# sauloal/pykmer

Measured on AMD Instinct MI355X. Metric: bp/s k-mer counted (k=15, 1 GPU), higher is better.
Workload: dtype u8; 1 GPU; k=15 canonical k-mer count of one 800 Mbp synthetic genome per GPU (SURVEY 8d C2, seed 2+rank), 4^15 table resident in HBM; fasta_bytes=813333854, num_kmers=766212116, parallelism=1 independent genome(s)

## Files before the change

### include/pykmer_hip.h

```cpp
#ifndef PYKMER_HIP_H
#define PYKMER_HIP_H

#include <stddef.h>
#include <stdint.h>

#ifdef __cplusplus
extern "C" {
#endif

#define PK_ABI_VERSION 3

enum {
    PK_OK = 0,
    PK_ERR_ARG = -1,
    PK_ERR_HIP = -2,
    PK_ERR_RECS_CAP = -3,
    PK_ERR_STATE = -4,
    PK_ERR_FORMAT = -5
};

#define PK_FORMAT_FASTA 0
#define PK_FORMAT_FASTQ 1

typedef struct pk_record {
// ... 114 lines not shown
int pk_trim_set_cover(pk_trim *t, const uint8_t *cover, uint64_t n_bases, int min_qual_byte);
int pk_trim_feed(pk_trim *t, const uint8_t *host_text, uint64_t n_bytes, const uint64_t *starts, uint64_t n_records, uint64_t *out);
int pk_trim_feed_device(pk_trim *t, const void *dev_text, uint64_t n_bytes, const uint64_t *starts, uint64_t n_records, uint64_t *out);
int pk_trim_finish(pk_trim *t, uint64_t totals_out[3]);
int pk_trim_timings(pk_trim *t, double out[2]);
void pk_trim_destroy(pk_trim *t);

enum { PK_CORR_POS2 = 0, PK_CORR_SEQ_LEN = 1, PK_CORR_CANDIDATES = 2, PK_CORR_UNTRIED = 3, PK_CORR_CORRECTED = 4, PK_CORR_AMBIGUOUS = 5,
       PK_CORR_FIELDS = 6 };
typedef struct pk_correct pk_correct;
int pk_correct_create(pk_correct **out, int k, int device);
int pk_correct_set_tables(pk_correct *c, const void *const *dev_tables, int N, int min_count, int max_count);
int pk_correct_set_cover(pk_correct *c, const uint8_t *cover, uint64_t n_bases, int min_qual_byte, int min_windows);
int pk_correct_feed(pk_correct *c, const uint8_t *host_text, uint64_t n_bytes, const uint64_t *starts, uint64_t n_records,
                    uint8_t *host_text_out, uint64_t *out);
int pk_correct_feed_device(pk_correct *c, const void *dev_text, uint64_t n_bytes, const uint64_t *starts, uint64_t n_records,
                           void *dev_text_out, uint64_t *out);
int pk_correct_finish(pk_correct *c, uint64_t totals_out[6]);
int pk_correct_timings(pk_correct *c, double out[2]);
void pk_correct_destroy(pk_correct *c);

int pk_bgzf_scan(const uint8_t *src, uint64_t n_bytes, uint64_t cap, uint64_t *c_off_out, uint64_t *c_size_out,
                 uint64_t *isize_out, uint64_t *n_blocks_out);
int pk_bgzf_inflate(const uint8_t *src, uint64_t src_bytes, const uint64_t *c_off, const uint64_t *c_size,
                    const uint64_t *u_off, uint64_t n_blocks, uint8_t *dst, int threads);
int pk_bgzf_deflate(const uint8_t *src, uint64_t n_bytes, int level, uint32_t block_input, uint8_t *dst, uint64_t dst_cap,
                    uint64_t *c_sizes_out, uint64_t *total_out, int threads);

int pk_diag_occupancy(int which);
int pk_diag_plan(int k, uint64_t n_bytes, uint64_t out[8]);
int pk_diag_settled_chunks(pk_indexer *ix, uint64_t *out);
int pk_diag_plan_slice(int k, int n_slices, uint64_t n_bytes, uint64_t out[16]);
int pk_diag_level2_order(const uint32_t *sizes, uint32_t B1, uint32_t *order_out);

#ifdef __cplusplus
}
#endif
#endif
```

### pykmer_amd/_lib.py

```python
import ctypes
import os

import numpy as np

_HERE = os.path.dirname(os.path.abspath(__file__))
from ._rt import LIB_PATH, open_library

PK_OK, PK_ERR_ARG, PK_ERR_HIP, PK_ERR_RECS_CAP, PK_ERR_STATE, PK_ERR_FORMAT = 0, -1, -2, -3, -4, -5
PK_FORMAT_FASTA, PK_FORMAT_FASTQ = 0, 1
FORMATS = {"fasta": PK_FORMAT_FASTA, "fastq": PK_FORMAT_FASTQ}
MASK_HARD, MASK_INVERT = 1, 2

RECORD_DTYPE = np.dtype([("name_off", "<u8"), ("name_len", "<u8"), ("seq_len", "<u8"), ("n_valid_kmers", "<u8")])

_u64p = ctypes.POINTER(ctypes.c_uint64)
_SIGNATURES = {
    "pk_version": (ctypes.c_int, []),
    "pk_last_error": (ctypes.c_int, [ctypes.c_char_p, ctypes.c_size_t]),
    "pk_device_count": (ctypes.c_int, []),
    "pk_warm": (ctypes.c_int, [ctypes.c_int]),
    "pk_dev_alloc": (ctypes.c_int, [ctypes.POINTER(ctypes.c_void_p), ctypes.c_uint64, ctypes.c_int]),
    "pk_dev_free": (ctypes.c_int, [ctypes.c_void_p, ctypes.c_int]),
    "pk_dev_upload": (ctypes.c_int, [ctypes.c_void_p, ctypes.c_void_p, ctypes.c_uint64, ctypes.c_int]),
    "pk_dev_download": (ctypes.c_int, [ctypes.c_void_p, ctypes.c_void_p, ctypes.c_uint64, ctypes.c_int]),
# ... 66 lines not shown
    "pk_select_set_records": (ctypes.c_int, [ctypes.c_void_p, ctypes.c_void_p, ctypes.c_void_p, ctypes.c_uint64]),
    "pk_select_feed": (ctypes.c_int, [ctypes.c_void_p, ctypes.c_void_p, ctypes.c_uint64, ctypes.c_void_p, ctypes.c_uint64, _u64p]),
    "pk_select_feed_device": (ctypes.c_int, [ctypes.c_void_p, ctypes.c_void_p, ctypes.c_uint64, ctypes.c_void_p, ctypes.c_uint64, _u64p]),
    "pk_select_finish": (ctypes.c_int, [ctypes.c_void_p, ctypes.c_void_p]),
    "pk_select_timings": (ctypes.c_int, [ctypes.c_void_p, ctypes.c_void_p]),
    "pk_select_destroy": (None, [ctypes.c_void_p]),
    "pk_trim_create": (ctypes.c_int, [ctypes.POINTER(ctypes.c_void_p), ctypes.c_int]),
    "pk_trim_set_cover": (ctypes.c_int, [ctypes.c_void_p, ctypes.c_void_p, ctypes.c_uint64, ctypes.c_int]),
    "pk_trim_feed": (ctypes.c_int, [ctypes.c_void_p, ctypes.c_void_p, ctypes.c_uint64, ctypes.c_void_p, ctypes.c_uint64, ctypes.c_void_p]),
    "pk_trim_feed_device": (ctypes.c_int, [ctypes.c_void_p, ctypes.c_void_p, ctypes.c_uint64, ctypes.c_void_p, ctypes.c_uint64, ctypes.c_void_p]),
    "pk_trim_finish": (ctypes.c_int, [ctypes.c_void_p, ctypes.c_void_p]),
    "pk_trim_timings": (ctypes.c_int, [ctypes.c_void_p, ctypes.c_void_p]),
    "pk_trim_destroy": (None, [ctypes.c_void_p]),
    "pk_correct_create": (ctypes.c_int, [ctypes.POINTER(ctypes.c_void_p), ctypes.c_int, ctypes.c_int]),
    "pk_correct_set_tables": (ctypes.c_int, [ctypes.c_void_p, ctypes.c_void_p, ctypes.c_int, ctypes.c_int, ctypes.c_int]),
    "pk_correct_set_cover": (ctypes.c_int, [ctypes.c_void_p, ctypes.c_void_p, ctypes.c_uint64, ctypes.c_int, ctypes.c_int]),
    "pk_correct_feed": (ctypes.c_int, [ctypes.c_void_p, ctypes.c_void_p, ctypes.c_uint64, ctypes.c_void_p, ctypes.c_uint64, ctypes.c_void_p,
                                        ctypes.c_void_p]),
    "pk_correct_feed_device": (ctypes.c_int, [ctypes.c_void_p, ctypes.c_void_p, ctypes.c_uint64, ctypes.c_void_p, ctypes.c_uint64, ctypes.c_void_p,
                                               ctypes.c_void_p]),
    "pk_correct_finish": (ctypes.c_int, [ctypes.c_void_p, ctypes.c_void_p]),
    "pk_correct_timings": (ctypes.c_int, [ctypes.c_void_p, ctypes.c_void_p]),
    "pk_correct_destroy": (None, [ctypes.c_void_p]),
    "pk_bgzf_scan": (ctypes.c_int, [ctypes.c_void_p, ctypes.c_uint64, ctypes.c_uint64, ctypes.c_void_p, ctypes.c_void_p, ctypes.c_void_p, _u64p]),
    "pk_bgzf_inflate": (ctypes.c_int, [ctypes.c_void_p, ctypes.c_uint64, ctypes.c_void_p, ctypes.c_void_p, ctypes.c_void_p, ctypes.c_uint64, ctypes.c_void_p,
                                        ctypes.c_int]),
    "pk_bgzf_deflate": (ctypes.c_int, [ctypes.c_void_p, ctypes.c_uint64, ctypes.c_int, ctypes.c_uint32, ctypes.c_void_p, ctypes.c_uint64,
                                        ctypes.c_void_p, _u64p, ctypes.c_int]),
    "pk_diag_occupancy": (ctypes.c_int, [ctypes.c_int]),
    "pk_diag_plan": (ctypes.c_int, [ctypes.c_int, ctypes.c_uint64, ctypes.c_void_p]),
    "pk_diag_settled_chunks": (ctypes.c_int, [ctypes.c_void_p, _u64p]),
    "pk_diag_plan_slice": (ctypes.c_int, [ctypes.c_int, ctypes.c_int, ctypes.c_uint64, ctypes.c_void_p]),
    "pk_diag_level2_order": (ctypes.c_int, [ctypes.c_void_p, ctypes.c_uint32, ctypes.c_void_p]),
}
EXPORTS = tuple(_SIGNATURES)

_lib = None


class PkError(RuntimeError):
    def __init__(self, code, message):
        super().__init__(f"libpykmer_hip error {code}: {message}")
        self.code = code


def load():
    global _lib
    if _lib is None:
        lib = open_library()
        for name, (res, args) in _SIGNATURES.items():
            fn = getattr(lib, name)
            fn.restype, fn.argtypes = res, args
        _lib = lib
    return _lib


def _check(rc):
    if rc != PK_OK:
        buf = ctypes.create_string_buffer(512)
        load().pk_last_error(buf, 512)
        msg = buf.value.decode("utf-8", "replace")
        if rc == PK_ERR_ARG:
            raise ValueError(msg)
        raise PkError(rc, msg)


# ... 646 lines not shown
                                  ctypes.byref(total), int(threads)))
    return dst[: total.value], sizes[:n_blocks].astype(np.int64)


def diag_plan(k: int, n_bytes: int = 0) -> dict:
    out = np.zeros(8, dtype=np.uint64)
    _check(load().pk_diag_plan(k, n_bytes, out.ctypes.data))
    names = ("feed_max", "capacity1", "capacity2", "B1", "B2", "fb_bits", "n_chunks", "fits_u32")
    return {n: int(v) for n, v in zip(names, out)}


WS_VARIANTS = ("narrow", "narrow_sliced", "k15", "k17", "wide_sliced", "deep", "wide")
COUNT_KERNELS = ("whole", "bytes", "half")


def diag_plan_slice(k: int, n_slices: int = 1, n_bytes: int = 0) -> dict:
    out = np.zeros(16, dtype=np.uint64)
    _check(load().pk_diag_plan_slice(k, n_slices, n_bytes, out.ctypes.data))
    names = ("addr_bits", "fb_bits", "b1", "b2", "sample_stride", "n_tally", "sample2", "n_chunks", "variant", "count_kernel",
             "split", "B1", "B2", "capacity1", "capacity2", "fits_u32")
    d = {n: int(v) for n, v in zip(names, out)}
    d["variant"] = WS_VARIANTS[d["variant"]]
    d["count_kernel"] = COUNT_KERNELS[d["count_kernel"]]
    return d


def diag_level2_order(sizes) -> np.ndarray:
    s = np.ascontiguousarray(sizes, dtype=np.uint32)
    out = np.zeros(max(1, s.size), dtype=np.uint32)
    _check(load().pk_diag_level2_order(s.ctypes.data, s.size, out.ctypes.data))
    return out[:s.size]


def gram_expand(pair: np.ndarray) -> np.ndarray:
    p = np.ascontiguousarray(pair, dtype=np.uint64)
    N = p.shape[0]
    m = np.zeros((N, N, 3), dtype=np.uint64)
    _check(load().pk_gram_expand(p.ctypes.data, N, m.ctypes.data))
    return m
```

### pykmer_amd/csrc/kmer_part.hip

```cpp
#include <cstddef>
#include <string>
#include <type_traits>
#include "../../include/pykmer_hip.h"
#include "part_common.h"

namespace pk {

int set_error(int code, const std::string &msg);

__global__ __launch_bounds__(1024) void k_sample2(const uint32_t *__restrict__ in, const uint32_t *__restrict__ bucket_base,
                                                  const uint32_t *__restrict__ bucket_end, PartPlan pl, uint32_t stride2,
                                                  uint32_t *__restrict__ tally, uint32_t *__restrict__ sampled_n,
                                                  const uint32_t *__restrict__ flags) {
    __shared__ uint32_t h[512];
    __shared__ uint32_t n_seen;
    if (flags[0]) return;
    const uint32_t b = blockIdx.x, lo = bucket_base[b], hi = bucket_end[b];
    if (threadIdx.x < 512) h[threadIdx.x] = 0;
    if (threadIdx.x == 0) n_seen = 0;
    __syncthreads();
    const uint32_t n_grp = (hi - lo + 255u) / 256u, n_sgrp = (n_grp + stride2 - 1u) / stride2;
    const uint32_t mask = pl.B2 - 1u, shift = pl.fb_bits, w = threadIdx.x >> 6, lane = threadIdx.x & 63u;
    uint32_t mine = 0;
    for (uint32_t s0 = 0; s0 < n_sgrp; s0 += 8u * 16u) {
// ... 138 lines not shown
            }
            const bool full = v_lo == win && n_tile == (uint32_t)TILE;
            uint32_t okm = 0;
            if (!full) {
#pragma unroll
                for (int j = 0; j < PER / 4; j++) {
                    const uint32_t i = win + (threadIdx.x + j * NT) * 4u;
#pragma unroll
                    for (int e = 0; e < 4; e++) okm |= (i + e >= v_lo && i + e < v_hi) ? (1u << (j * 4 + e)) : 0u;
                }
            }
            if (win + TILE < hi) fetch(win + TILE, nxt);
            uint32_t *cl = cursor + (uint64_t)b * B;
            const uint32_t *ce = cap_end + (uint64_t)b * B;
            if (full) scatter_tile<uint32_t, false, NT, PER, 512, true, 8, REC24>(L, r, 0u, n_tile, shift, B, low_mask, true, out, settle, cl, ce, dump, flags);
            else scatter_tile<uint32_t, false, NT, PER, 512, false, 8, REC24>(L, r, okm, n_tile, shift, B, low_mask, true, out, settle, cl, ce, dump, flags);
        }
    };
    const uint32_t *pos = wg2_start;
    const uint32_t per = pl.B1 >> 3;
    const uint32_t o_lo = (blockIdx.x & 7u) * per, o_hi = o_lo + per, first = blockIdx.x >> 3, step = gridDim.x >> 3;
    const uint32_t w_end = pos[o_hi];
    for (uint32_t w = pos[o_lo] + first; w < w_end; w += step) {
        uint32_t a = o_lo, z = o_hi;
        while (z - a > 1) { const uint32_t m = (a + z) >> 1; if (pos[m] <= w) a = m; else z = m; }
        const uint32_t b = l2_order[a];
        const uint64_t s = (uint64_t)bucket_base[b] + (uint64_t)(w - pos[a]) * pl.R2;
        const uint64_t e = min(s + pl.R2, (uint64_t)bucket_end[b]);
        item(b, (uint32_t)s, (uint32_t)e);
    }
}

constexpr uint32_t K6_PIECE = 65024;
constexpr int K6_BYTES_LDS = 65536 + 1024 + 128;

__device__ __forceinline__ int wave_sum_i32(int v) {
    v += __builtin_amdgcn_update_dpp(0, v, 0x128, 0xf, 0xf, false);
    v += __builtin_amdgcn_update_dpp(0, v, 0x124, 0xf, 0xf, false);
    v += __builtin_amdgcn_update_dpp(0, v, 0x122, 0xf, 0xf, false);
    v += __builtin_amdgcn_update_dpp(0, v, 0x121, 0xf, 0xf, false);
    return __builtin_amdgcn_readlane(v, 0) + __builtin_amdgcn_readlane(v, 16) + __builtin_amdgcn_readlane(v, 32) +
           __builtin_amdgcn_readlane(v, 48);
}

typedef unsigned short U16x2 __attribute__((ext_vector_type(2)));
__device__ __forceinline__ uint32_t clamp255_pair(uint32_t x) {
    const U16x2 lim = {255, 255};
    return __builtin_bit_cast(uint32_t, __builtin_elementwise_min(__builtin_bit_cast(U16x2, x), lim));
}
__device__ __forceinline__ uint32_t pack_low_bytes(uint32_t x0, uint32_t x1) {
    return __builtin_amdgcn_perm(x1, x0, 0x06040200u);
}

struct SliceTally {
    int d1 = 0, d2 = 0;
    __device__ __forceinline__ void add_dword(int *dh, uint32_t x, int sign) {
        uint32_t p0 = x & 0x01010101u, p1 = (x >> 1) & 0x01010101u;
        uint32_t rest = p0 & p1;
        const uint32_t high = x & 0xfcfcfcfcu;
        if (high) {
            const uint32_t big = (((high & 0x7f7f7f7fu) + 0x7f7f7f7fu) | high) & 0x80808080u;
            const uint32_t keep = ~(big >> 7);
            p0 &= keep; p1 &= keep;
            rest = (p0 & p1) | (big >> 7);
        }
        const int n1 = (int)__builtin_popcount(p0 & ~p1), n2 = (int)__builtin_popcount(p1 & ~p0);
        d1 += sign * n1; d2 += sign * n2;
        while (rest) {
            const int bit = __ffs(rest) - 1;
            atomicAdd(&dh[(x >> bit) & 0xffu], sign);
            rest &= rest - 1u;
        }
    }
};

template <int T, bool LEAN, bool NOREC = false>
__device__ __forceinline__ void bucket_count_body(const uint16_t *__restrict__ recs, const uint32_t *__restrict__ final_start,
                                                  const uint32_t *__restrict__ final_end, uint32_t fb_bits, uint32_t split_bits,
                                                  uint8_t *__restrict__ table8, uint32_t fresh, unsigned long long *__restrict__ hist_rep, uint8_t *smem,
                                                  int *dh, uint32_t wg) {
    uint32_t *cnt = reinterpret_cast<uint32_t *>(smem);
    const uint32_t fb = wg >> split_bits, part = wg & ((1u << split_bits) - 1u);
    const uint32_t start = final_start[fb], end = final_end ? final_end[fb] : final_start[fb + 1];
    const uint32_t part_bits = fb_bits - split_bits;
    const uint32_t n_addr = 1u << part_bits;
    uint8_t *slice = table8 + ((uint64_t)fb << fb_bits) + (uint64_t)part * n_addr;
    if (start == end) {
        if (fresh) {
            if (n_addr >= 16) for (uint32_t g = threadIdx.x; g < n_addr / 16; g += T) reinterpret_cast<uint4 *>(slice)[g] = make_uint4(0, 0, 0, 0);
            else for (uint32_t a = threadIdx.x; a < n_addr; a += T) slice[a] = 0;
        }
        return;
    }
    const uint32_t base = start & ~7u;
    const uint32_t i_first = base + threadIdx.x * 8;
    uint4 v_first = make_uint4(0, 0, 0, 0);
    if (i_first < min(base + K6_PIECE, end)) v_first = *reinterpret_cast<const uint4 *>(recs + i_first);
    const bool by_rec = NOREC ? false : (((end - start) >> split_bits) < n_addr / 4 || n_addr < 16);
    SliceTally tally;
    for (uint32_t i = threadIdx.x; i < 256; i += T) dh[i] = 0;
    if (fresh) {
        if (n_addr >= 8) for (uint32_t g = threadIdx.x; g < n_addr / 8; g += T) reinterpret_cast<uint4 *>(cnt)[g] = make_uint4(0, 0, 0, 0);
        else for (uint32_t a = threadIdx.x; a < max(n_addr / 2, 1u); a += T) cnt[a] = 0u;
    } else if (n_addr >= 16) {
        if (!by_rec) __syncthreads();
        for (uint32_t g = threadIdx.x; g < n_addr / 16; g += T) {
            uint4 v = reinterpret_cast<const uint4 *>(slice)[g];
            uint32_t w[4] = {v.x, v.y, v.z, v.w};
            if (!by_rec) {
#pragma unroll
                for (int q = 0; q < 4; q++) tally.add_dword(dh, w[q], -1);
            }
#pragma unroll
            for (int q = 0; q < 8; q++)
                cnt[g * 8 + q] = __builtin_amdgcn_perm(0u, w[q >> 1], (q & 1) ? 0x0c030c02u : 0x0c010c00u);
        }
    } else {
        for (uint32_t a = threadIdx.x; a < max(n_addr / 2, 1u); a += T) cnt[a] = slice[2 * a] | (n_addr > 1u ? (uint32_t)slice[2 * a + 1] << 16 : 0u);
    }
    __syncthreads();
    auto bump = [&](uint32_t a, uint32_t n) {
        const uint32_t sh = 16u * (a & 1u);
        if (!by_rec) { atomicAdd(&cnt[a >> 1], n << sh); return; }
        int &d1 = tally.d1, &d2 = tally.d2;
        const uint32_t c = (atomicAdd(&cnt[a >> 1], n << sh) >> sh) & 0xffffu;
        const uint32_t oc = c > 255u ? 255u : c, nc = c + n > 255u ? 255u : c + n;
        if (oc == nc) return;
        if (nc == 1u) d1++;
        else if (nc == 2u && oc == 1u) { d2++; d1--; }
        else {
            atomicAdd(&dh[nc], 1);
            if (oc) atomicAdd(&dh[oc], -1);
        }
    };
    auto count8 = [&](const uint4 &v, uint32_t i) {
        const uint32_t w[4] = {v.x, v.y, v.z, v.w};
        if (LEAN && !by_rec) {
            const bool interior = i >= start && i + 8u <= end;
            uint8_t *cb = reinterpret_cast<uint8_t *>(cnt);
#pragma unroll
            for (int q = 0; q < 8; q++) {
                const uint32_t x = w[q >> 1];
                const uint32_t off = (q & 1) ? ((x >> 15) & 0x1fffcu) : ((x << 1) & 0x1fffcu);
                const uint32_t low = (q & 1) ? ((x >> 16) & 1u) : (x & 1u);
                uint32_t val = low * 0xffffu + 1u;
                if (!interior) val = (i + q >= start && i + q < end) ? val : 0u;
                __hip_atomic_fetch_add(reinterpret_cast<uint32_t *>(cb + off), val, __ATOMIC_RELAXED, __HIP_MEMORY_SCOPE_WORKGROUP);
            }
            return;
// ... 34 lines not shown
            else if (c == 1u) { tally.d2++; tally.d1--; }
            else { atomicAdd(&dh[c + 1u], 1); atomicAdd(&dh[c], -1); }
        }
    };
    constexpr int NIT = (K6_PIECE + T * 8 - 1) / (T * 8);
    if (end - base <= (uint32_t)T * 8u) {
        if (i_first < end) { if (by_rec) count8_sparse(v_first, i_first); else count8(v_first, i_first); }
        __syncthreads();
    } else {
        for (uint32_t p0 = base; p0 < end; p0 += K6_PIECE) {
            const uint32_t p1 = min(p0 + K6_PIECE, end);
            uint4 v[NIT];
#pragma unroll
            for (int it = 0; it < NIT; it++) {
                const uint32_t i = p0 + (threadIdx.x + it * T) * 8;
                v[it] = make_uint4(0, 0, 0, 0);
                if (i < p1) v[it] = (it == 0 && p0 == base) ? v_first : *reinterpret_cast<const uint4 *>(recs + i);
            }
#pragma unroll
            for (int it = 0; it < NIT; it++) {
                const uint32_t i = p0 + (threadIdx.x + it * T) * 8;
                if (i < p1) count8(v[it], i);
            }
            __syncthreads();
            if (p1 < end) {
                for (uint32_t a = threadIdx.x; a < max(n_addr / 2, 1u); a += T) {
                    cnt[a] = clamp255_pair(cnt[a]);
                }
                __syncthreads();
            }
        }
    }
    if (n_addr >= 16) {
        for (uint32_t g = threadIdx.x; g < n_addr / 16; g += T) {
            const uint4 c0 = reinterpret_cast<const uint4 *>(cnt)[g * 2], c1 = reinterpret_cast<const uint4 *>(cnt)[g * 2 + 1];
            const uint32_t o[4] = {pack_low_bytes(clamp255_pair(c0.x), clamp255_pair(c0.y)), pack_low_bytes(clamp255_pair(c0.z), clamp255_pair(c0.w)),
                                   pack_low_bytes(clamp255_pair(c1.x), clamp255_pair(c1.y)), pack_low_bytes(clamp255_pair(c1.z), clamp255_pair(c1.w))};
            if (!by_rec) {
#pragma unroll
                for (int q = 0; q < 4; q++) tally.add_dword(dh, o[q], 1);
            }
            reinterpret_cast<uint4 *>(slice)[g] = make_uint4(o[0], o[1], o[2], o[3]);
        }
    } else {
        for (uint32_t a = threadIdx.x; a < max(n_addr / 2, 1u); a += T) {
            uint32_t x = cnt[a], lo = x & 0xffffu, hi = x >> 16;
            slice[2 * a] = (uint8_t)(lo > 255u ? 255u : lo);
            if (n_addr > 1u) slice[2 * a + 1] = (uint8_t)(hi > 255u ? 255u : hi);
        }
    }
    const int d1 = wave_sum_i32(tally.d1), d2 = wave_sum_i32(tally.d2);
    if ((threadIdx.x & 63) == 0) {
        if (d1) atomicAdd(&dh[1], d1);
        if (d2) atomicAdd(&dh[2], d2);
    }
    __syncthreads();
    for (uint32_t i = threadIdx.x; i < 256; i += T) {
        const int v = dh[i];
        if (v) atomicAdd(&hist_rep[(uint64_t)(blockIdx.x % HIST_REPLICAS) * 256 + i], (unsigned long long)(long long)v);
    }
}

template <int T>
__global__ __launch_bounds__(T) void k_bucket_count(const uint16_t *__restrict__ recs, const uint32_t *__restrict__ final_start,
                                                    const uint32_t *__restrict__ final_end, uint32_t fb_bits, uint32_t split_bits,
                                                    uint8_t *__restrict__ table8, uint32_t fresh, unsigned long long *__restrict__ hist_rep,
                                                    const uint32_t *__restrict__ flags) {
    extern __shared__ __attribute__((aligned(16))) uint8_t smem[];
    __shared__ int dh[256];
    if (flags[0]) return;
    bucket_count_body<T, true>(recs, final_start, final_end, fb_bits, split_bits, table8, fresh, hist_rep, smem, dh, blockIdx.x);
}
template <int T, bool FRESH>
__global__ __launch_bounds__(T) __attribute__((amdgpu_waves_per_eu(8, 8)))
void k_bucket_count_half_lean(const uint16_t *__restrict__ recs, const uint32_t *__restrict__ final_start, const uint32_t *__restrict__ final_end,
                              uint32_t fb_bits, uint32_t split_bits, uint8_t *__restrict__ table8, uint32_t fresh, unsigned long long *__restrict__ hist_rep,
                              const uint32_t *__restrict__ flags) {
    extern __shared__ __attribute__((aligned(16))) uint8_t smem[];
    __shared__ int dh[256];
    if (flags[0]) return;
    bucket_count_body<T, true, true>(recs, final_start, final_end, 15u, 0u, table8, FRESH ? 1u : 0u, hist_rep, smem, dh, blockIdx.x);
}

template <int T>
__global__ __launch_bounds__(T) __attribute__((amdgpu_waves_per_eu(8, 8)))
void k_bucket_count_bytes(const uint16_t *__restrict__ recs, const uint32_t *__restrict__ final_start, const uint32_t *__restrict__ final_end,
                          uint8_t *__restrict__ table8, uint32_t fresh, unsigned long long *__restrict__ hist_rep,
                          const uint32_t *__restrict__ flags) {
    extern __shared__ __attribute__((aligned(128))) uint8_t smem[];
    constexpr uint32_t N_ADDR = 65536u;
    int *dh = reinterpret_cast<int *>(smem + N_ADDR);
    uint32_t *wrap_flag = reinterpret_cast<uint32_t *>(smem + N_ADDR + 1024);
    if (flags[0]) return;
    const uint32_t fb = blockIdx.x;
    const uint32_t start = final_start[fb], end = final_end ? final_end[fb] : final_start[fb + 1];
    uint4 *slice = reinterpret_cast<uint4 *>(table8 + ((uint64_t)fb << 16));
    uint4 *img = reinterpret_cast<uint4 *>(smem);
    if (start == end) {
        if (fresh) for (uint32_t g = threadIdx.x; g < N_ADDR / 16; g += T) slice[g] = make_uint4(0, 0, 0, 0);
        return;
    }
    bool recount = end - start >= 16384u;
    int d1 = 0, d2 = 0;
    if (!recount) {
        const uint32_t base = start & ~7u;
        const uint32_t i_first = base + threadIdx.x * 8;
        uint4 v = make_uint4(0, 0, 0, 0);
        if (i_first < end) v = *reinterpret_cast<const uint4 *>(recs + i_first);
        for (uint32_t i = threadIdx.x; i < 256; i += T) dh[i] = 0;
        if (threadIdx.x == 0) *wrap_flag = 0u;
        if (fresh) { for (uint32_t g = threadIdx.x; g < N_ADDR / 16; g += T) img[g] = make_uint4(0, 0, 0, 0); }
        else { for (uint32_t g = threadIdx.x; g < N_ADDR / 16; g += T) img[g] = slice[g]; }
        __syncthreads();
        uint32_t *cnt = reinterpret_cast<uint32_t *>(smem);
        bool wrapped = false;
        for (uint32_t p0 = base; p0 < end; p0 += (uint32_t)T * 8u) {
            const uint32_t i = p0 + threadIdx.x * 8;
            if (i >= end) continue;
            if (p0 != base) v = *reinterpret_cast<const uint4 *>(recs + i);
            const uint32_t w[4] = {v.x, v.y, v.z, v.w};
            const bool interior = i >= start && i + 8u <= end;
            uint32_t old[8];
            bool in[8];
#pragma unroll
            for (int q = 0; q < 8; q++) {
                const uint32_t a = (w[q >> 1] >> (16 * (q & 1))) & 0xffffu, sh = 8u * (a & 3u);
                in[q] = interior || (i + q >= start && i + q < end);
                old[q] = (atomicAdd(&cnt[a >> 2], in[q] ? (1u << sh) : 0u) >> sh) & 0xffu;
            }
#pragma unroll
            for (int q = 0; q < 8; q++) {
                const uint32_t c = old[q];
                if (!in[q]) continue;
                if (c == 0u) d1++;
                else if (c == 1u) { d2++; d1--; }
                else if (c == 255u) wrapped = true;
                else { atomicAdd(&dh[c + 1u], 1); atomicAdd(&dh[c], -1); }
            }
        }
        if (wrapped) *wrap_flag = 1u;
        __syncthreads();
        recount = *wrap_flag != 0u;
        __syncthreads();
    }
    if (recount) {
        if (threadIdx.x == 0) atomicAdd(const_cast<uint32_t *>(&flags[1]), 1u);
        bucket_count_body<T, false>(recs, final_start, final_end, 16u, 1u, table8, fresh, hist_rep, smem, dh, 2u * fb);
        __syncthreads();
        bucket_count_body<T, false>(recs, final_start, final_end, 16u, 1u, table8, fresh, hist_rep, smem, dh, 2u * fb + 1u);
        return;
    }
    for (uint32_t g = threadIdx.x; g < N_ADDR / 16; g += T) slice[g] = img[g];
    d1 = wave_sum_i32(d1); d2 = wave_sum_i32(d2);
    if ((threadIdx.x & 63) == 0) {
        if (d1) atomicAdd(&dh[1], d1);
        if (d2) atomicAdd(&dh[2], d2);
    }
    __syncthreads();
    for (uint32_t i = threadIdx.x; i < 256; i += T) {
        const int x = dh[i];
        if (x) atomicAdd(&hist_rep[(uint64_t)(blockIdx.x % HIST_REPLICAS) * 256 + i], (unsigned long long)(long long)x);
    }
}

__device__ __forceinline__ void hist_reduce(unsigned long long *__restrict__ hist_rep, unsigned long long *__restrict__ hist) {
    if (threadIdx.x >= 256) return;
    unsigned long long acc = 0;
    for (uint32_t r = 0; r < HIST_REPLICAS; r++) {
        acc += hist_rep[(uint64_t)r * 256 + threadIdx.x];
        hist_rep[(uint64_t)r * 256 + threadIdx.x] = 0ull;
    }
    if (acc) atomicAdd(&hist[threadIdx.x], acc);
}

constexpr uint32_t AS_SLOTS = 4096, AS_WGS = 64;

__device__ __forceinline__ void table_sat_add(uint8_t *table8, uint64_t addr, uint32_t cnt, int *dh) {
    unsigned int *word = reinterpret_cast<unsigned int *>(table8 + (addr & ~3ull));
    const uint32_t sh = (uint32_t)(addr & 3ull) * 8u;
    unsigned int old = *word;
    while (true) {
        uint32_t b = (old >> sh) & 0xffu;
// ... 139 lines not shown
    b.side_n = &b.signals->side_n;
    b.flags = b.signals->flags;
    return o;
}

void part_set_attributes() {
    fuse_set_attributes();
    hipFuncSetAttribute((const void *)k_scatter2<512, 32>, hipFuncAttributeMaxDynamicSharedMemorySize, (int)SCATTER_LDS_NARROW);
    hipFuncSetAttribute((const void *)k_scatter2<512, 32, true>, hipFuncAttributeMaxDynamicSharedMemorySize, (int)SCATTER_LDS_NARROW);
    hipFuncSetAttribute((const void *)k_bucket_count<1024>, hipFuncAttributeMaxDynamicSharedMemorySize, 128 * 1024);
    hipFuncSetAttribute((const void *)k_bucket_count_half_lean<1024, true>, hipFuncAttributeMaxDynamicSharedMemorySize, 128 * 1024);
    hipFuncSetAttribute((const void *)k_bucket_count_half_lean<1024, false>, hipFuncAttributeMaxDynamicSharedMemorySize, 128 * 1024);
    hipFuncSetAttribute((const void *)k_bucket_count_bytes<1024>, hipFuncAttributeMaxDynamicSharedMemorySize, K6_BYTES_LDS);
}

extern "C" int pk_diag_occupancy(int which) {
    int n = -1;
    hipError_t e = hipErrorInvalidValue;
    if (which == 0) e = hipOccupancyMaxActiveBlocksPerMultiprocessor(&n, (const void *)k_bucket_count<1024>, 1024, 128 * 1024);
    if (which == 1) e = hipOccupancyMaxActiveBlocksPerMultiprocessor(&n, (const void *)k_bucket_count_bytes<1024>, 1024, K6_BYTES_LDS);
    if (which == 2) e = hipOccupancyMaxActiveBlocksPerMultiprocessor(&n, (const void *)k_bucket_count_half_lean<1024, true>, 1024, 65536);
    if (which == 3) e = hipOccupancyMaxActiveBlocksPerMultiprocessor(&n, (const void *)k_scatter2<512, 32>, 512, SCATTER_LDS_NARROW);
    return e == hipSuccess ? n : -(int)e;
}

extern "C" int pk_diag_level2_order(const uint32_t *sizes, uint32_t B1, uint32_t *order_out) {
    if (!sizes || !order_out) return set_error(PK_ERR_ARG, "pk_diag_level2_order: null argument");
    static_assert(PART_MAX_B1 == 512, "the message below and include/pykmer_hip.h name the limit");
    if (B1 < 8u || B1 > PART_MAX_B1 || (B1 & 7u)) return set_error(PK_ERR_ARG, "pk_diag_level2_order: B1 must be a multiple of 8 from 8 to 512");
    for (uint32_t b = 0; b < B1; b++) order_out[level2_position(level2_rank(sizes, B1, b), B1)] = b;
    return PK_OK;
}

int launch_partitioned(const PartPlan &pl, const PartBuffers &b, const L2 *st2, uint64_t n_bytes, uint32_t stride, const Carry *carry, uint8_t *table8,
                       unsigned long long *hist, unsigned long long *hist_rep, bool fresh, const PartEvents &ev, hipStream_t s) {
    const uint32_t nfb = pl.B1 * pl.B2;
    const uint32_t *flags = b.flags;
    const char *failed = nullptr;
    hipError_t why = hipSuccess;
    const auto stage = [&](const char *name) { if (!failed && (why = hipGetLastError()) != hipSuccess) failed = name; };
    launch_provision(pl, b, st2, stride, carry, s);
    stage("bucket layout");
    hipEventRecord(ev.sort_begin, s);
    launch_walk_sort(pl, b, st2, carry, s);
    stage("level-1 sort");
    hipEventRecord(ev.sort_end, s);
    const uint16_t *final_recs = (const uint16_t *)b.out1;
    const uint32_t *k6_start = b.bucket_base, *k6_end = b.bucket_end;
    if (pl.sample2) {
        const uint32_t stride2 = stride == 1u ? 1u : 16u, n_blocks = (nfb + 1023u) / 1024u;
        const uint32_t *base1 = b.bucket_base, *end1 = b.bucket_end;
        hipLaunchKernelGGL(k_sample2, dim3(pl.B1), dim3(1024), 0, s, (const uint32_t *)b.out1, base1, end1, pl, stride2, b.tally_tot, b.sampled_n, flags);
        hipLaunchKernelGGL(k_rooms2, dim3(n_blocks), dim3(1024), 0, s, (const uint32_t *)b.tally_tot, (const uint32_t *)b.sampled_n, base1, end1, pl, stride2,
                           nfb, b.final_start, b.cap2_end, b.block_tot, flags);
        hipLaunchKernelGGL(k_bases2, dim3(1), dim3(1024), 0, s, n_blocks, nfb, pl, b.block_tot, b.final_start, b.flags);
        hipLaunchKernelGGL(k_starts2, dim3(n_blocks), dim3(1024), 0, s, nfb, (const uint32_t *)b.block_tot, b.final_start, b.cursor2, b.cap2_end, flags);
        stage("final-bucket rooms");
    }
    if (pl.b2) {
        const uint32_t grid2 = 4096u;
        hipLaunchKernelGGL((pl.k <= 15 ? &k_scatter2<512, 32, true> : &k_scatter2<512, 32>), dim3(grid2), dim3(512), SCATTER_LDS_NARROW, s,
                           (const uint32_t *)b.out1, b.wg2_start, (const uint32_t *)b.l2_order, b.bucket_base, b.bucket_end, pl, b.out2, b.cursor2, (const uint32_t *)b.cap2_end,
                           (uint32_t)pl.capacity2, b.flags);
        stage("level 2");
        final_recs = (const uint16_t *)b.out2; k6_start = b.final_start; k6_end = b.cursor2;
    }
// ... 24 lines not shown
```

### pykmer_amd/csrc/part_common.h

```cpp
#pragma once
#include <cstddef>
#include "fasta_fsm.h"
#include "pk_kernels.h"

namespace pk {

constexpr int SC_T = 1024;
constexpr int SC_PER = 16;
constexpr int TILE = SC_T * SC_PER;

constexpr uint32_t HOT_PROBES = 16;
constexpr uint32_t SIDE_CNT_BITS = 28;

template <uint32_t SLOTS>
struct HotTable {
    static constexpr uint32_t HOT_SLOTS = SLOTS;
    unsigned long long key[SLOTS];
    uint32_t val[SLOTS];
    uint32_t used, n_flush;
    unsigned long long flush_base;
};

__device__ __forceinline__ void side_append_one(unsigned long long *side, unsigned long long *side_n, uint64_t side_cap,
                                                uint64_t addr, uint32_t cnt) {
// ... 28 lines not shown
    __syncthreads();
    uint32_t mine = 0;
    for (uint32_t i = threadIdx.x; i < HOT_SLOTS; i += blockDim.x) mine += H.key[i] != 0ull;
    uint32_t at = mine ? atomicAdd(&H.n_flush, mine) : 0u;
    __syncthreads();
    if (threadIdx.x == 0) H.flush_base = H.n_flush ? atomicAdd(side_n, (unsigned long long)H.n_flush) : 0ull;
    __syncthreads();
    const unsigned long long base64 = H.flush_base;
    for (uint32_t i = threadIdx.x; i < HOT_SLOTS; i += blockDim.x) {
        if (H.key[i] != 0ull) {
            unsigned long long dst = base64 + at++;
            if (dst < side_cap) side[dst] = ((H.key[i] - 1ull) << SIDE_CNT_BITS) | H.val[i];
            H.key[i] = 0ull; H.val[i] = 0u;
        }
    }
    if (threadIdx.x == 0) H.used = 0;
    __syncthreads();
}


__host__ __device__ __forceinline__ size_t level1_hi_plane_offset(uint64_t capacity1) {
    return (((size_t)(capacity1 + TILE + 64) * 2u) + 255u) & ~(size_t)255u;
}

__host__ __device__ __forceinline__ uint32_t level2_rank(const uint32_t *sizes, uint32_t B1, uint32_t b) {
    const uint32_t mine = sizes[b];
    uint32_t rank = 0;
    for (uint32_t j = 0; j < B1; j++) rank += (sizes[j] > mine || (sizes[j] == mine && j < b)) ? 1u : 0u;
    return rank;
}
__host__ __device__ __forceinline__ uint32_t level2_position(uint32_t rank, uint32_t B1) {
    const uint32_t round = rank >> 3, c = rank & 7u;
    return ((round & 1u) ? 7u - c : c) * (B1 >> 3) + round;
}

__device__ __forceinline__ uint32_t wave_incl_scan_u32(uint32_t v) {
    v += (uint32_t)__builtin_amdgcn_update_dpp(0, (int)v, 0x111, 0xf, 0xf, false);
    v += (uint32_t)__builtin_amdgcn_update_dpp(0, (int)v, 0x112, 0xf, 0xf, false);
    v += (uint32_t)__builtin_amdgcn_update_dpp(0, (int)v, 0x114, 0xf, 0xf, false);
    v += (uint32_t)__builtin_amdgcn_update_dpp(0, (int)v, 0x118, 0xf, 0xf, false);
    v += (uint32_t)__builtin_amdgcn_update_dpp(0, (int)v, 0x142, 0xa, 0xf, false);
    v += (uint32_t)__builtin_amdgcn_update_dpp(0, (int)v, 0x143, 0xc, 0xf, false);
    return v;
}

template <int NB>
struct ScatterLdsT {
    uint32_t hist[NB + 64], off[NB + 64], run[NB], gbase[NB];
    uint32_t wsum[SC_T / 64];
    uint32_t total, pad_[3];
    uint32_t rec[TILE + 64];
    uint16_t dig[TILE + 64];
};
typedef ScatterLdsT<512> ScatterLds;
constexpr size_t SCATTER_LDS_NARROW = offsetof(ScatterLds, dig);
constexpr size_t SCATTER_LDS_WIDE = sizeof(ScatterLds);

template <typename RIN, bool WIDE, int NT = SC_T, int PER = SC_PER, int NB = 512, bool FULL = false, int SB = 0, bool OFF32 = false, class Settle>
__device__ __forceinline__ void scatter_tile(ScatterLdsT<NB> &L, const RIN (&r)[PER], uint32_t okm, uint32_t n_tile,
                                             uint32_t shift, uint32_t B, uint32_t low_mask, bool out16, void *__restrict__ out,
                                             Settle &&settle, uint32_t *claim = nullptr, const uint32_t *__restrict__ cap_end = nullptr,
                                             uint32_t dump = 0, uint32_t *overflow = nullptr, uint8_t *__restrict__ out_hi = nullptr,
                                             const uint32_t *watch = nullptr, uint32_t watch_limit = 0,
                                             bool *watch_hit = nullptr) {
    static_assert(NT * PER == TILE, "tile shape");
    const uint32_t lane = threadIdx.x & 63u;
// ... 141 lines not shown
```

Baseline: 225.9 billion bp/s.

## Tally slice count deltas via byte moment sums and wave-queued big bytes

Replaces the per-dword popcount and serial atomic loop in the slice histogram tally with algebraic byte moments (popcount, sum via sad_u8, sum of squares via udot4). The counts of values 1, 2 and 3 are then recovered per wave from those moments. Bytes of 4 or more are compacted through a per-wave LDS queue using ballot/mbcnt and drained 64 at a time, so the histogram atomics run with the wave fully active rather than in divergent per-lane loops. Loops are padded to wave multiples so the wave-synchronous drains stay uniform. This costs extra LDS for the queues, which may reduce occupancy, and adds a host-side diagnostic entry point.

```diff
diff --git a/include/pykmer_hip.h b/include/pykmer_hip.h
--- a/include/pykmer_hip.h
+++ b/include/pykmer_hip.h
@@ -170,6 +170,7 @@
 int pk_diag_settled_chunks(pk_indexer *ix, uint64_t *out);
 int pk_diag_plan_slice(int k, int n_slices, uint64_t n_bytes, uint64_t out[16]);
 int pk_diag_level2_order(const uint32_t *sizes, uint32_t B1, uint32_t *order_out);
+int pk_diag_slice_tally(const uint8_t *stored, const uint8_t *loaded, uint32_t n_bytes, int32_t counts_out[3]);
 
 #ifdef __cplusplus
 }
diff --git a/pykmer_amd/_lib.py b/pykmer_amd/_lib.py
--- a/pykmer_amd/_lib.py
+++ b/pykmer_amd/_lib.py
@@ -122,6 +122,7 @@
     "pk_diag_settled_chunks": (ctypes.c_int, [ctypes.c_void_p, _u64p]),
     "pk_diag_plan_slice": (ctypes.c_int, [ctypes.c_int, ctypes.c_int, ctypes.c_uint64, ctypes.c_void_p]),
     "pk_diag_level2_order": (ctypes.c_int, [ctypes.c_void_p, ctypes.c_uint32, ctypes.c_void_p]),
+    "pk_diag_slice_tally": (ctypes.c_int, [ctypes.c_void_p, ctypes.c_void_p, ctypes.c_uint32, ctypes.c_void_p]),
 }
 EXPORTS = tuple(_SIGNATURES)
 
@@ -834,6 +835,16 @@
     return out[:s.size]
 
 
+def diag_slice_tally(stored, loaded=None) -> np.ndarray:
+    s = np.ascontiguousarray(stored, dtype=np.uint8)
+    ld = None if loaded is None else np.ascontiguousarray(loaded, dtype=np.uint8)
+    if ld is not None and ld.size != s.size:
+        raise ValueError("diag_slice_tally: the two slices differ in length")
+    out = np.zeros(3, dtype=np.int32)
+    _check(load().pk_diag_slice_tally(s.ctypes.data, None if ld is None else ld.ctypes.data, s.size, out.ctypes.data))
+    return out
+
+
 def gram_expand(pair: np.ndarray) -> np.ndarray:
     p = np.ascontiguousarray(pair, dtype=np.uint64)
     N = p.shape[0]
diff --git a/pykmer_amd/csrc/kmer_part.hip b/pykmer_amd/csrc/kmer_part.hip
--- a/pykmer_amd/csrc/kmer_part.hip
+++ b/pykmer_amd/csrc/kmer_part.hip
@@ -194,7 +194,8 @@
 }
 
 constexpr uint32_t K6_PIECE = 65024;
-constexpr int K6_BYTES_LDS = 65536 + 1024 + 128;
+constexpr uint32_t TALLY_QUEUE = 128;
+constexpr int K6_BYTES_LDS = 65536 + 1024 + 128 + 1024 / 64 * TALLY_QUEUE * 4;
 
 __device__ __forceinline__ int wave_sum_i32(int v) {
     v += __builtin_amdgcn_update_dpp(0, v, 0x128, 0xf, 0xf, false);
@@ -214,25 +215,50 @@
     return __builtin_amdgcn_perm(x1, x0, 0x06040200u);
 }
 
+__device__ __forceinline__ void tally_wave_sync() {
+    __builtin_amdgcn_fence(__ATOMIC_RELEASE, "wavefront");
+    __builtin_amdgcn_wave_barrier();
+    __builtin_amdgcn_fence(__ATOMIC_ACQUIRE, "wavefront");
+}
+
 struct SliceTally {
     int d1 = 0, d2 = 0;
-    __device__ __forceinline__ void add_dword(int *dh, uint32_t x, int sign) {
-        uint32_t p0 = x & 0x01010101u, p1 = (x >> 1) & 0x01010101u;
-        uint32_t rest = p0 & p1;
-        const uint32_t high = x & 0xfcfcfcfcu;
-        if (high) {
-            const uint32_t big = (((high & 0x7f7f7f7fu) + 0x7f7f7f7fu) | high) & 0x80808080u;
-            const uint32_t keep = ~(big >> 7);
-            p0 &= keep; p1 &= keep;
-            rest = (p0 & p1) | (big >> 7);
-        }
-        const int n1 = (int)__builtin_popcount(p0 & ~p1), n2 = (int)__builtin_popcount(p1 & ~p0);
-        d1 += sign * n1; d2 += sign * n2;
-        while (rest) {
-            const int bit = __ffs(rest) - 1;
-            atomicAdd(&dh[(x >> bit) & 0xffu], sign);
-            rest &= rest - 1u;
-        }
+    ByteSums sums;
+    uint32_t fill = 0;
+
+    __device__ __forceinline__ void drain(uint32_t *queue, int *dh, int sign, uint32_t first, uint32_t n) {
+        const uint32_t lane = threadIdx.x & 63u;
+        tally_wave_sync();
+        const uint32_t e = lane < n ? queue[first + lane] : 0u;
+        tally_wave_sync();
+        const uint32_t high = e & 0xfcfcfcfcu;
+        const uint32_t big = (((high & 0x7f7f7f7fu) + 0x7f7f7f7fu) | high) & 0x80808080u;
+        byte_sums_add<true>(sums, e & ((big - (big >> 7)) | big));
+#pragma unroll
+        for (int j = 0; j < 4; j++) {
+            const uint32_t b = (e >> (8 * j)) & 0xffu;
+            if (b >= 4u) atomicAdd(&dh[b], sign);
+        }
+    }
+    __device__ __forceinline__ void add_dword(uint32_t *queue, int *dh, uint32_t x, int sign) {
+        byte_sums_add(sums, x);
+        const bool big = (x & 0xfcfcfcfcu) != 0u;
+        const unsigned long long m = __builtin_amdgcn_ballot_w64(big);
+        if (m) {
+            if (big) queue[fill + __builtin_amdgcn_mbcnt_hi((uint32_t)(m >> 32), __builtin_amdgcn_mbcnt_lo((uint32_t)m, 0u))] = x;
+            fill += (uint32_t)__popcll(m);
+            if (fill >= 64u) { fill -= 64u; drain(queue, dh, sign, fill, 64u); }
+        }
+    }
+    __device__ __forceinline__ void end_phase(uint32_t *queue, int *dh, int sign) {
+        if (fill) drain(queue, dh, sign, 0u, fill);
+        fill = 0u;
+    }
+    __device__ __forceinline__ ByteSums wave_sums(bool take) {
+        ByteSums w;
+        w.p = (uint32_t)wave_sum_i32((int)sums.p); w.s1 = (uint32_t)wave_sum_i32((int)sums.s1); w.s2 = (uint32_t)wave_sum_i32((int)sums.s2);
+        if (take) sums = ByteSums();
+        return w;
     }
 };
 
@@ -240,8 +266,9 @@
 __device__ __forceinline__ void bucket_count_body(const uint16_t *__restrict__ recs, const uint32_t *__restrict__ final_start,
                                                   const uint32_t *__restrict__ final_end, uint32_t fb_bits, uint32_t split_bits,
                                                   uint8_t *__restrict__ table8, uint32_t fresh, unsigned long long *__restrict__ hist_rep, uint8_t *smem,
-                                                  int *dh, uint32_t wg) {
+                                                  int *dh, uint32_t *tally_queue, uint32_t wg) {
     uint32_t *cnt = reinterpret_cast<uint32_t *>(smem);
+    uint32_t *queue = tally_queue + (threadIdx.x >> 6) * TALLY_QUEUE;
     const uint32_t fb = wg >> split_bits, part = wg & ((1u << split_bits) - 1u);
     const uint32_t start = final_start[fb], end = final_end ? final_end[fb] : final_start[fb + 1];
     const uint32_t part_bits = fb_bits - split_bits;
@@ -260,23 +287,29 @@
     if (i_first < min(base + K6_PIECE, end)) v_first = *reinterpret_cast<const uint4 *>(recs + i_first);
     const bool by_rec = NOREC ? false : (((end - start) >> split_bits) < n_addr / 4 || n_addr < 16);
     SliceTally tally;
+    ByteSums loaded;
     for (uint32_t i = threadIdx.x; i < 256; i += T) dh[i] = 0;
     if (fresh) {
         if (n_addr >= 8) for (uint32_t g = threadIdx.x; g < n_addr / 8; g += T) reinterpret_cast<uint4 *>(cnt)[g] = make_uint4(0, 0, 0, 0);
         else for (uint32_t a = threadIdx.x; a < max(n_addr / 2, 1u); a += T) cnt[a] = 0u;
     } else if (n_addr >= 16) {
         if (!by_rec) __syncthreads();
-        for (uint32_t g = threadIdx.x; g < n_addr / 16; g += T) {
-            uint4 v = reinterpret_cast<const uint4 *>(slice)[g];
+        for (uint32_t g = threadIdx.x; g < ((n_addr / 16 + 63u) & ~63u); g += T) {
+            const bool in = g < n_addr / 16;
+            uint4 v = make_uint4(0, 0, 0, 0);
+            if (in) v = reinterpret_cast<const uint4 *>(slice)[g];
             uint32_t w[4] = {v.x, v.y, v.z, v.w};
             if (!by_rec) {
 #pragma unroll
-                for (int q = 0; q < 4; q++) tally.add_dword(dh, w[q], -1);
-            }
-#pragma unroll
-            for (int q = 0; q < 8; q++)
-                cnt[g * 8 + q] = __builtin_amdgcn_perm(0u, w[q >> 1], (q & 1) ? 0x0c030c02u : 0x0c010c00u);
-        }
+                for (int q = 0; q < 4; q++) tally.add_dword(queue, dh, w[q], -1);
+            }
+            if (in) {
+#pragma unroll
+                for (int q = 0; q < 8; q++)
+                    cnt[g * 8 + q] = __builtin_amdgcn_perm(0u, w[q >> 1], (q & 1) ? 0x0c030c02u : 0x0c010c00u);
+            }
+        }
+        if (!by_rec) { tally.end_phase(queue, dh, -1); loaded = tally.wave_sums(true); }
     } else {
         for (uint32_t a = threadIdx.x; a < max(n_addr / 2, 1u); a += T) cnt[a] = slice[2 * a] | (n_addr > 1u ? (uint32_t)slice[2 * a + 1] << 16 : 0u);
     }
@@ -377,16 +410,19 @@
         }
     }
     if (n_addr >= 16) {
-        for (uint32_t g = threadIdx.x; g < n_addr / 16; g += T) {
-            const uint4 c0 = reinterpret_cast<const uint4 *>(cnt)[g * 2], c1 = reinterpret_cast<const uint4 *>(cnt)[g * 2 + 1];
+        for (uint32_t g = threadIdx.x; g < ((n_addr / 16 + 63u) & ~63u); g += T) {
+            const bool in = g < n_addr / 16;
+            uint4 c0 = make_uint4(0, 0, 0, 0), c1 = c0;
+            if (in) { c0 = reinterpret_cast<const uint4 *>(cnt)[g * 2]; c1 = reinterpret_cast<const uint4 *>(cnt)[g * 2 + 1]; }
             const uint32_t o[4] = {pack_low_bytes(clamp255_pair(c0.x), clamp255_pair(c0.y)), pack_low_bytes(clamp255_pair(c0.z), clamp255_pair(c0.w)),
                                    pack_low_bytes(clamp255_pair(c1.x), clamp255_pair(c1.y)), pack_low_bytes(clamp255_pair(c1.z), clamp255_pair(c1.w))};
             if (!by_rec) {
 #pragma unroll
-                for (int q = 0; q < 4; q++) tally.add_dword(dh, o[q], 1);
-            }
-            reinterpret_cast<uint4 *>(slice)[g] = make_uint4(o[0], o[1], o[2], o[3]);
-        }
+                for (int q = 0; q < 4; q++) tally.add_dword(queue, dh, o[q], 1);
+            }
+            if (in) reinterpret_cast<uint4 *>(slice)[g] = make_uint4(o[0], o[1], o[2], o[3]);
+        }
+        if (!by_rec) tally.end_phase(queue, dh, 1);
     } else {
         for (uint32_t a = threadIdx.x; a < max(n_addr / 2, 1u); a += T) {
             uint32_t x = cnt[a], lo = x & 0xffffu, hi = x >> 16;
@@ -394,10 +430,21 @@
             if (n_addr > 1u) slice[2 * a + 1] = (uint8_t)(hi > 255u ? 255u : hi);
         }
     }
-    const int d1 = wave_sum_i32(tally.d1), d2 = wave_sum_i32(tally.d2);
-    if ((threadIdx.x & 63) == 0) {
-        if (d1) atomicAdd(&dh[1], d1);
-        if (d2) atomicAdd(&dh[2], d2);
+    if (by_rec) {
+        const int d1 = wave_sum_i32(tally.d1), d2 = wave_sum_i32(tally.d2);
+        if ((threadIdx.x & 63) == 0) {
+            if (d1) atomicAdd(&dh[1], d1);
+            if (d2) atomicAdd(&dh[2], d2);
+        }
+    } else {
+        ByteSums w = tally.wave_sums(false);
+        w.p -= loaded.p; w.s1 -= loaded.s1; w.s2 -= loaded.s2;
+        if ((threadIdx.x & 63) == 0) {
+            int n[3];
+            byte_sums_counts(w, n);
+#pragma unroll
+            for (int v = 0; v < 3; v++) if (n[v]) atomicAdd(&dh[v + 1], n[v]);
+        }
     }
     __syncthreads();
     for (uint32_t i = threadIdx.x; i < 256; i += T) {
@@ -413,8 +460,9 @@
                                                     const uint32_t *__restrict__ flags) {
     extern __shared__ __attribute__((aligned(16))) uint8_t smem[];
     __shared__ int dh[256];
+    __shared__ uint32_t tally_queue[T / 64 * TALLY_QUEUE];
     if (flags[0]) return;
-    bucket_count_body<T, true>(recs, final_start, final_end, fb_bits, split_bits, table8, fresh, hist_rep, smem, dh, blockIdx.x);
+    bucket_count_body<T, true>(recs, final_start, final_end, fb_bits, split_bits, table8, fresh, hist_rep, smem, dh, tally_queue, blockIdx.x);
 }
 template <int T, bool FRESH>
 __global__ __launch_bounds__(T) __attribute__((amdgpu_waves_per_eu(8, 8)))
@@ -423,8 +471,9 @@
                               const uint32_t *__restrict__ flags) {
     extern __shared__ __attribute__((aligned(16))) uint8_t smem[];
     __shared__ int dh[256];
+    __shared__ uint32_t tally_queue[T / 64 * TALLY_QUEUE];
     if (flags[0]) return;
-    bucket_count_body<T, true, true>(recs, final_start, final_end, 15u, 0u, table8, FRESH ? 1u : 0u, hist_rep, smem, dh, blockIdx.x);
+    bucket_count_body<T, true, true>(recs, final_start, final_end, 15u, 0u, table8, FRESH ? 1u : 0u, hist_rep, smem, dh, tally_queue, blockIdx.x);
 }
 
 template <int T>
@@ -436,6 +485,7 @@
     constexpr uint32_t N_ADDR = 65536u;
     int *dh = reinterpret_cast<int *>(smem + N_ADDR);
     uint32_t *wrap_flag = reinterpret_cast<uint32_t *>(smem + N_ADDR + 1024);
+    uint32_t *tally_queue = reinterpret_cast<uint32_t *>(smem + N_ADDR + 1024 + 128);
     if (flags[0]) return;
     const uint32_t fb = blockIdx.x;
     const uint32_t start = final_start[fb], end = final_end ? final_end[fb] : final_start[fb + 1];
@@ -490,9 +540,9 @@
     }
     if (recount) {
         if (threadIdx.x == 0) atomicAdd(const_cast<uint32_t *>(&flags[1]), 1u);
-        bucket_count_body<T, false>(recs, final_start, final_end, 16u, 1u, table8, fresh, hist_rep, smem, dh, 2u * fb);
+        bucket_count_body<T, false>(recs, final_start, final_end, 16u, 1u, table8, fresh, hist_rep, smem, dh, tally_queue, 2u * fb);
         __syncthreads();
-        bucket_count_body<T, false>(recs, final_start, final_end, 16u, 1u, table8, fresh, hist_rep, smem, dh, 2u * fb + 1u);
+        bucket_count_body<T, false>(recs, final_start, final_end, 16u, 1u, table8, fresh, hist_rep, smem, dh, tally_queue, 2u * fb + 1u);
         return;
     }
     for (uint32_t g = threadIdx.x; g < N_ADDR / 16; g += T) slice[g] = img[g];
@@ -698,6 +748,25 @@
     return PK_OK;
 }
 
+extern "C" int pk_diag_slice_tally(const uint8_t *stored, const uint8_t *loaded, uint32_t n_bytes, int32_t counts_out[3]) {
+    if (!stored || !counts_out) return set_error(PK_ERR_ARG, "pk_diag_slice_tally: null argument");
+    if ((n_bytes & 3u) || n_bytes > 65536u) return set_error(PK_ERR_ARG, "pk_diag_slice_tally: n_bytes must be a multiple of 4, at most 65536");
+    ByteSums sums;
+    for (int pass = 0; pass < 2; pass++) {
+        const uint8_t *slice = pass ? stored : loaded;
+        for (uint32_t i = 0; slice && i < n_bytes; i += 4) {
+            const uint32_t x = (uint32_t)slice[i] | (uint32_t)slice[i + 1] << 8 | (uint32_t)slice[i + 2] << 16 | (uint32_t)slice[i + 3] << 24;
+            if (x & 0xfcfcfcfcu) return set_error(PK_ERR_ARG, "pk_diag_slice_tally: a byte above 3");
+            byte_sums_add(sums, x);
+        }
+        if (!pass) { sums.p = 0u - sums.p; sums.s1 = 0u - sums.s1; sums.s2 = 0u - sums.s2; }
+    }
+    int counts[3];
+    byte_sums_counts(sums, counts);
+    for (int v = 0; v < 3; v++) counts_out[v] = counts[v];
+    return PK_OK;
+}
+
 int launch_partitioned(const PartPlan &pl, const PartBuffers &b, const L2 *st2, uint64_t n_bytes, uint32_t stride, const Carry *carry, uint8_t *table8,
                        unsigned long long *hist, unsigned long long *hist_rep, bool fresh, const PartEvents &ev, hipStream_t s) {
     const uint32_t nfb = pl.B1 * pl.B2;
diff --git a/pykmer_amd/csrc/part_common.h b/pykmer_amd/csrc/part_common.h
--- a/pykmer_amd/csrc/part_common.h
+++ b/pykmer_amd/csrc/part_common.h
@@ -84,6 +84,35 @@
 __host__ __device__ __forceinline__ uint32_t level2_position(uint32_t rank, uint32_t B1) {
     const uint32_t round = rank >> 3, c = rank & 7u;
     return ((round & 1u) ? 7u - c : c) * (B1 >> 3) + round;
+}
+
+struct ByteSums { uint32_t p = 0, s1 = 0, s2 = 0; };
+
+template <bool SUB = false>
+__host__ __device__ __forceinline__ void byte_sums_add(ByteSums &s, uint32_t x) {
+#if defined(__HIP_DEVICE_COMPILE__)
+    if (!SUB) {
+        s.p += (uint32_t)__builtin_popcount(x);
+        s.s1 = __builtin_amdgcn_sad_u8(x, 0u, s.s1);
+        s.s2 = __builtin_amdgcn_udot4(x, x, s.s2, false);
+    } else {
+        s.p -= (uint32_t)__builtin_popcount(x);
+        s.s1 -= __builtin_amdgcn_sad_u8(x, 0u, 0u);
+        s.s2 -= __builtin_amdgcn_udot4(x, x, 0u, false);
+    }
+#else
+    for (int j = 0; j < 4; j++) {
+        const uint32_t b = (x >> (8 * j)) & 0xffu;
+        const uint32_t p = (uint32_t)__builtin_popcount(b);
+        s.p += SUB ? 0u - p : p; s.s1 += SUB ? 0u - b : b; s.s2 += SUB ? 0u - b * b : b * b;
+    }
+#endif
+}
+__host__ __device__ __forceinline__ void byte_sums_counts(const ByteSums &s, int counts[3]) {
+    const uint32_t a = s.s1 - s.p, b = s.s2 - s.s1;
+    const int n3 = (int)(b - 2u * a) / 4;
+    const int n2 = (int)a - n3;
+    counts[0] = (int)s.p - n2 - 2 * n3; counts[1] = n2; counts[2] = n3;
 }
 
 __device__ __forceinline__ uint32_t wave_incl_scan_u32(uint32_t v) {
```

Measured after the change: 226.0 billion bp/s, median of 2. About the same (+0.0%).
